# Improbable-AI/walk-these-ways

Hardware: AMD Instinct MI355X
Metric: env-steps/sec (sim+PPO) (higher is better)
Workload: dtype f32

## Files before the change

include/go1ppo.h:

```cpp
#ifndef GO1PPO_H
#define GO1PPO_H
#include <stdint.h>

#ifdef __cplusplus
extern "C" {
#endif

#define GO1PPO_ABI_VERSION 3
#define GO1PPO_MAX_ACTIONS 32

int go1ppo_elu_fwd(void* y, int64_t rows, int cols, int ld, const void* lat, int lat_ld, int npv, const void* wz,
                   int wz_ld, int lat_cols, void* stream);

int go1ppo_elu_bwd(const void* d, int ld_d, const void* h, int ld_h, int64_t rows, int cols, float* bias_grad, void* out,
                   int ld_out, void* stream);

typedef struct {
  const void* mean;
  const void* value;
  const float* std;
  int32_t head_ld, num_actions;
  int64_t rows;
  const int64_t* idx;
  const float* actions;
// ... 3 lines not shown
  const float* advantages;
  const float* returns;
  const float* old_values;
  float clip_param, value_loss_coef, entropy_coef;
  int32_t use_clipped_value_loss;
  void* d_mean;
  void* d_value;
  float* d_std;
  float* d_mean_bias;
  float* d_value_bias;
  float* kl;
  float* value_loss;
  float* surrogate_loss;
} Go1PpoLossArgs;

int go1ppo_loss(const Go1PpoLossArgs* args, void* stream);

int go1ppo_mse(const void* pred, int pred_ld, const float* target, int npv, const int64_t* idx, int64_t rows,
               int64_t num_train, int selective, void* d_pred, float* d_pred_bias, float* train_loss,
               float* test_loss, void* stream);

int go1ppo_wgrad(const void* dz, int ld_dz, const void* h, int ld_h, int64_t rows, int n, int k, float* dW, int ldw,
                 float* bias_grad, void* stream);

#define GO1PPO_TAIL_MAX_LAYERS 4
#define GO1PPO_TAIL_MAX_NETS 3
typedef struct {
  const void* W;
  const void* bias;
  void* out;
  int32_t n_out, k_in, ld_out, elu;
} Go1PpoTailLayer;
typedef struct {
  const void* in;
  int64_t rows;
  int32_t ld_in, num_layers;
  int32_t elu_in, npv;
  const void* latent;
  const void* wz;
  int32_t lat_ld, wz_ld;
  Go1PpoTailLayer layer[GO1PPO_TAIL_MAX_LAYERS];
} Go1PpoTailNet;
typedef struct {
  int32_t num_nets, _pad;
  Go1PpoTailNet net[GO1PPO_TAIL_MAX_NETS];
} Go1PpoTailArgs;
int go1ppo_tail_fwd(const Go1PpoTailArgs* args, void* stream);

typedef struct {
  const void* dz;
  const void* h;
  float* dW;
  float* bias_grad;
  int64_t rows;
  int32_t ld_dz, ld_h, n, k, ldw;
  int32_t chunk_rows, wg_offset;
  int32_t zero_n, zero_k0, zero_k1;
  float* partials;
  int64_t partial_stride;
} Go1PpoWgradProblem;

int go1ppo_wgrad_plan(Go1PpoWgradProblem* host_problems, int count);
int go1ppo_wgrad_batched(const Go1PpoWgradProblem* device_problems, int count, int total_workgroups, void* stream);


int go1ppo_act(const void* mean, const void* value, int head_ld, const float* std, int num_actions, int64_t rows,
               const float* noise, float* actions, float* mu, float* sigma, float* values, float* logp, void* stream);

int go1ppo_store_step(const float* rewards, const uint8_t* dones, const uint8_t* time_outs, const int32_t* env_bins,
                      const float* values, float gamma, int64_t n, float* rewards_out, uint8_t* dones_out,
                      float* env_bins_out, void* stream);

int go1ppo_gae(const float* rewards, const uint8_t* dones, const float* values, const float* last_values, int T, int64_t N,
               float gamma, float lam, float* returns, float* advantages, double* stats, void* stream);

int go1ppo_normalize(float* adv, int64_t n, const double* stats, void* stream);


int go1ppo_ring_snapshot(const float* hist, int64_t ld_hist, int64_t N, int H, int no, void* ring, void* stream);

int go1ppo_ring_step(const float* obs, const float* priv, void* ring_dst, const void* ring_window, int64_t N, int H, int no,
                     int npv, int Kp, void* X, float* obs_store, float* priv_store, void* stream);

int go1ppo_ring_gather(const void* ring, const float* priv_store, const int64_t* idx, int64_t rows, int64_t N, int H, int no,
                       int npv, int Kp, void* X, void* stream);


int go1ppo_opt_partials(void);

int go1ppo_opt_prestep(const float* g, int64_t n, float gscale, float* partial, float* step, float* lr, const float* kl,
                       float kl_scale, float desired_kl, float lr_min, float lr_max, void* stream);

typedef struct {
  int64_t begin, count;
  const void* src;
  int64_t stride;
  int32_t kind, slabs, cols, zero_rows, zero_c0, zero_c1;
} Go1PpoGradPiece;
int go1ppo_grad_reduce(float* g, const Go1PpoGradPiece* device_pieces, int num_pieces, void* stream);
int go1ppo_opt_prestep_pieces(float* g, int64_t n, const Go1PpoGradPiece* device_pieces, int num_pieces, float gscale, float* partial,
                              float* step, float* lr, const float* kl, float kl_scale, float desired_kl, float lr_min, float lr_max,
                              void* stream);

#define GO1PPO_ADAM_MAX_TRANSPOSES 2
typedef struct {
  int32_t num_transposes, _pad;
  struct { int64_t start; int32_t rows, cols; void* dst; } transpose[GO1PPO_ADAM_MAX_TRANSPOSES];
// ... 52 lines not shown
```

walk-these-ways_amd/csrc/go1ppo_gemm.h:

```cpp
#pragma once

#define GEMM_BM 128
#define GEMM_BN 128
#define GEMM_BK 64

typedef __attribute__((address_space(3))) void lds_void_t;
typedef __attribute__((address_space(1))) const void global_cvoid_t;

__device__ __forceinline__ void glds16(const bf16_t* g, bf16_t* lds_wave_base) {
  __builtin_amdgcn_global_load_lds((global_cvoid_t*)g, (lds_void_t*)lds_wave_base, 16, 0, 0);
}

template <int EPI>
__device__ __forceinline__ void gemm_nt_body(const Go1PpoGemmArgs& a, bf16_t (*lds)[2][GEMM_BM * GEMM_BK]) {
  const int lane = threadIdx.x & 63, wave = threadIdx.x >> 6;
  const int nwg = gridDim.x, orig = blockIdx.x;
  const int q = nwg >> 3, r = nwg & 7, xcd = orig & 7;
  const int logical = (xcd < r ? xcd * (q + 1) : r * (q + 1) + (xcd - r) * q) + (orig >> 3);
  const int tiles_n = (a.N + GEMM_BN - 1) / GEMM_BN;
  const int m0 = (logical / tiles_n) * GEMM_BM, n0 = (logical % tiles_n) * GEMM_BN;

  const int srow = lane >> 3;
  const bf16_t* ga[4];
  const bf16_t* gb[4];
// ... 258 lines not shown
}
__device__ __forceinline__ bf16x8_t tn_operand(const TnFrags& f, int i) {
  s16x8_t v = __builtin_shufflevector(f.lo[i], f.hi[i], 0, 1, 2, 3, 4, 5, 6, 7);
  return __builtin_bit_cast(bf16x8_t, v);
}

#define WTN_T 128
#define WTN_STEP 64
#define WTN_BUFS 4
#define WTN_THREADS 512

__device__ __forceinline__ void wgrad_tn_body(const bf16_t* P, int ldp, const bf16_t* Q, int ldq, int64_t m_begin, int steps,
                                              float* C, int ldc, float* bias_row, int N, int K, int n0, int k0,
                                              bf16_t (*lds)[2][WTN_STEP * WTN_T], int zero_n, int zero_k0, int zero_k1, bool slab) {
  const int lane = threadIdx.x & 63, wave = threadIdx.x >> 6;
  const bf16_t* gp[2];
  const bf16_t* gq[2];
  bool vp[2], vq[2];
#pragma unroll
  for (int p = 0; p < 2; p++) {
    const int row = (wave * 2 + p) * 4 + (lane >> 4);
    const int chunk = (lane & 15) ^ (2 * ((row & 3) | (((row >> 3) & 1) << 2)));
    const int cn = n0 + chunk * 8, ck = k0 + chunk * 8;
    vp[p] = cn < N;
    vq[p] = ck < K;
    gp[p] = P + (m_begin + row) * ldp + (vp[p] ? cn : 0);
    gq[p] = Q + (m_begin + row) * ldq + (vq[p] ? ck : 0);
  }
  auto stage_piece = [&](int step, int p, int op) {
    const int buf = step & (WTN_BUFS - 1);
    if (op == 0) { if (vp[p]) glds16(gp[p] + (int64_t)step * WTN_STEP * ldp, &lds[buf][0][(wave * 2 + p) * 4 * WTN_T]); }
    else { if (vq[p]) glds16(gq[p] + (int64_t)step * WTN_STEP * ldq, &lds[buf][1][(wave * 2 + p) * 4 * WTN_T]); }
  };
  auto stage = [&](int step) {
    stage_piece(step, 0, 0); stage_piece(step, 0, 1); stage_piece(step, 1, 0); stage_piece(step, 1, 1);
  };
  const int g = lane >> 4, i16 = lane & 15;
  const int rowoff = (g * 8 + (i16 >> 2)) * 256 + ((i16 & 3) >> 1) * 16 + (i16 & 1) * 8;
  const int swb = 32 * ((i16 >> 2) | ((g & 1) << 2));
  const int wn = wave >> 2, wk = wave & 3;
  int fa[4], fb[2];
#pragma unroll
  for (int f = 0; f < 4; f++) fa[f] = rowoff + (((wn * 64 + f * 16) * 2) ^ swb);
#pragma unroll
  for (int f = 0; f < 2; f++) fb[f] = rowoff + (((wk * 32 + f * 16) * 2) ^ swb);
  f32x4 acc[4][2], bacc[4];
#pragma unroll
  for (int a = 0; a < 4; a++) {
    bacc[a] = f32x4{0.f, 0.f, 0.f, 0.f};
#pragma unroll
    for (int b = 0; b < 2; b++) acc[a][b] = f32x4{0.f, 0.f, 0.f, 0.f};
  }
  const bool do_bias = bias_row && k0 == 0 && wk == 0;
  const s16x8_t ones_bits = {0x3f80, 0x3f80, 0x3f80, 0x3f80, 0x3f80, 0x3f80, 0x3f80, 0x3f80};
  const bf16x8_t ones = __builtin_bit_cast(bf16x8_t, ones_bits);

  const uint32_t lds0 = (uint32_t)(uintptr_t)(lds_void_t*)&lds[0][0][0];
#pragma unroll
  for (int s = 0; s < WTN_BUFS - 1; s++)
    if (s < steps) stage(s);
  for (int s = 0; s < steps; s++) {
    const int younger = steps - 1 - s;
    if (younger >= 2) asm volatile("s_waitcnt vmcnt(8)" ::: "memory");
    else if (younger == 1) asm volatile("s_waitcnt vmcnt(4)" ::: "memory");
    else asm volatile("s_waitcnt vmcnt(0)" ::: "memory");
    __builtin_amdgcn_s_barrier();
    asm volatile("" ::: "memory");
    const bool more = s + WTN_BUFS - 1 < steps;
    const int nxt = s + WTN_BUFS - 1;
    const uint32_t base = lds0 + (uint32_t)(s & (WTN_BUFS - 1)) * (2 * WTN_STEP * WTN_T * 2);
    uint32_t aa[4], ab[2];
#pragma unroll
    for (int f = 0; f < 4; f++) aa[f] = base + fa[f];
#pragma unroll
    for (int f = 0; f < 2; f++) ab[f] = base + WTN_STEP * WTN_T * 2 + fb[f];
    TnFrags f0, f1;
    tn_read<0>(f0, aa, ab);
    tn_read<1>(f1, aa, ab);
    if (more) { stage_piece(nxt, 0, 0); stage_piece(nxt, 0, 1); }
    lds_wait<12>(f0);
#pragma unroll
    for (int a = 0; a < 4; a++) {
#pragma unroll
      for (int b = 0; b < 2; b++)
        acc[a][b] = __builtin_amdgcn_mfma_f32_16x16x32_bf16(tn_operand(f0, a), tn_operand(f0, 4 + b), acc[a][b], 0, 0, 0);
      if (a == 1 && more) stage_piece(nxt, 1, 0);
    }
    if (do_bias) {
#pragma unroll
      for (int a = 0; a < 4; a++) bacc[a] = __builtin_amdgcn_mfma_f32_16x16x32_bf16(tn_operand(f0, a), ones, bacc[a], 0, 0, 0);
    }
    if (more) stage_piece(nxt, 1, 1);
    lds_wait<0>(f1);
#pragma unroll
    for (int a = 0; a < 4; a++)
#pragma unroll
      for (int b = 0; b < 2; b++)
        acc[a][b] = __builtin_amdgcn_mfma_f32_16x16x32_bf16(tn_operand(f1, a), tn_operand(f1, 4 + b), acc[a][b], 0, 0, 0);
    if (do_bias) {
#pragma unroll
      for (int a = 0; a < 4; a++) bacc[a] = __builtin_amdgcn_mfma_f32_16x16x32_bf16(tn_operand(f1, a), ones, bacc[a], 0, 0, 0);
    }
  }
#pragma unroll
  for (int a = 0; a < 4; a++) {
#pragma unroll
    for (int e = 0; e < 4; e++) {
      const int n = n0 + wn * 64 + a * 16 + 4 * g + e;
      if (n >= N) continue;
#pragma unroll
      for (int b = 0; b < 2; b++) {
        const int k = k0 + wk * 32 + b * 16 + i16;
        if (k < K && !(n < zero_n && k >= zero_k0 && k < zero_k1)) {
          if (slab) C[(int64_t)n * ldc + k] = acc[a][b][e];
          else atomicAdd(C + (int64_t)n * ldc + k, acc[a][b][e]);
        }
      }
    }
    if (do_bias && i16 == 0 && n0 + wn * 64 + a * 16 + 4 * g < N) det_put4(bias_row, (wn * 64 + a * 16 + 4 * g) * (int)sizeof(float), bacc[a]);
  }
}

#define WTW_BUF_BYTES (3 * WTN_STEP * WTN_T * 2)
#define WTW_BUFS 3
struct TnFragsW { s16x4_t lo[8], hi[8]; };
template <int KK>
__device__ __forceinline__ void tnw_read(TnFragsW& f, const uint32_t (&aa)[4], const uint32_t (&ab)[4]) {
#pragma unroll
// ... 6 lines not shown
    f.lo[4 + i] = lds_tr<KK * 32 * 256>(ab[i]);
    f.hi[4 + i] = lds_tr<KK * 32 * 256 + 4 * 256>(ab[i]);
  }
}
__device__ __forceinline__ void ldsw_wait_all(TnFragsW& f) {
  asm volatile("s_waitcnt lgkmcnt(0)"
               : "+v"(f.lo[0]), "+v"(f.lo[1]), "+v"(f.lo[2]), "+v"(f.lo[3]), "+v"(f.lo[4]), "+v"(f.lo[5]), "+v"(f.lo[6]), "+v"(f.lo[7]));
  asm volatile("" : "+v"(f.hi[0]), "+v"(f.hi[1]), "+v"(f.hi[2]), "+v"(f.hi[3]), "+v"(f.hi[4]), "+v"(f.hi[5]), "+v"(f.hi[6]), "+v"(f.hi[7]));
}
__device__ __forceinline__ bf16x8_t tnw_operand(const TnFragsW& f, int i) {
  s16x8_t v = __builtin_shufflevector(f.lo[i], f.hi[i], 0, 1, 2, 3, 4, 5, 6, 7);
  return __builtin_bit_cast(bf16x8_t, v);
}

__device__ __forceinline__ void wgrad_tn_body_wide(const bf16_t* P, int ldp, const bf16_t* Q, int ldq, int64_t m_begin, int steps,
                                                   float* C, int ldc, float* bias_row, int N, int K, int n0, int k0, char* lds,
                                                   int zero_n, int zero_k0, int zero_k1, bool slab) {
  const int lane = threadIdx.x & 63, wave = threadIdx.x >> 6;
  const bf16_t* src[6];
  bool ok[6];
  int dst[6];
#pragma unroll
  for (int q = 0; q < 6; q++) {
    const int id = q < 4 ? wave * 4 + q : wave * 2 + (q - 4);
    const int img = q < 4 ? id >> 4 : 2, rb = q < 4 ? id & 15 : id;
    const int row = rb * 4 + (lane >> 4);
    const int chunk = (lane & 15) ^ (2 * ((row & 3) | (((row >> 3) & 1) << 2)));
    const int col = (q < 4 ? n0 + img * 128 : k0) + chunk * 8;
    ok[q] = col < (q < 4 ? N : K);
    src[q] = (q < 4 ? P + (m_begin + row) * ldp : Q + (m_begin + row) * ldq) + (ok[q] ? col : 0);
    dst[q] = img * (WTN_STEP * WTN_T * 2) + rb * 4 * WTN_T * 2;
  }
  auto stage_piece = [&](int step, int buf, int q) {
    if (ok[q]) glds16(src[q] + (int64_t)step * WTN_STEP * (q < 4 ? ldp : ldq), (bf16_t*)(lds + buf * WTW_BUF_BYTES + dst[q]));
  };
  const int g = lane >> 4, i16 = lane & 15;
  const int rowoff = (g * 8 + (i16 >> 2)) * 256 + ((i16 & 3) >> 1) * 16 + (i16 & 1) * 8;
  const int swb = 32 * ((i16 >> 2) | ((g & 1) << 2));
  const int wn = wave >> 1, wk = wave & 1;
  int fa[4], fb[4];
#pragma unroll
  for (int f = 0; f < 4; f++) {
    fa[f] = (wn >> 1) * (WTN_STEP * WTN_T * 2) + rowoff + ((((wn & 1) * 64 + f * 16) * 2) ^ swb);
    fb[f] = 2 * (WTN_STEP * WTN_T * 2) + rowoff + (((wk * 64 + f * 16) * 2) ^ swb);
  }
  f32x4 acc[4][4], bacc[4];
#pragma unroll
  for (int a = 0; a < 4; a++) {
    bacc[a] = f32x4{0.f, 0.f, 0.f, 0.f};
#pragma unroll
    for (int b = 0; b < 4; b++) acc[a][b] = f32x4{0.f, 0.f, 0.f, 0.f};
  }
  const bool do_bias = bias_row && k0 == 0 && wk == 0;
  const s16x8_t ones_bits = {0x3f80, 0x3f80, 0x3f80, 0x3f80, 0x3f80, 0x3f80, 0x3f80, 0x3f80};
  const bf16x8_t ones = __builtin_bit_cast(bf16x8_t, ones_bits);
  const uint32_t lds0 = (uint32_t)(uintptr_t)(lds_void_t*)lds;
#pragma unroll
  for (int s = 0; s < WTW_BUFS - 1; s++)
    if (s < steps) {
#pragma unroll
      for (int q = 0; q < 6; q++) stage_piece(s, s, q);
    }
  int buf = 0;
  for (int s = 0; s < steps; s++) {
    if (s + 1 < steps) asm volatile("s_waitcnt vmcnt(6)" ::: "memory");
    else asm volatile("s_waitcnt vmcnt(0)" ::: "memory");
    __builtin_amdgcn_s_barrier();
    asm volatile("" ::: "memory");
    const bool more = s + WTW_BUFS - 1 < steps;
    const int nxt = s + WTW_BUFS - 1, nbuf = buf == 0 ? WTW_BUFS - 1 : buf - 1;
    const uint32_t base = lds0 + (uint32_t)buf * WTW_BUF_BYTES;
    uint32_t aa[4], ab[4];
#pragma unroll
    for (int f = 0; f < 4; f++) { aa[f] = base + fa[f]; ab[f] = base + fb[f]; }
    TnFragsW f0, f1;
    tnw_read<0>(f0, aa, ab);
    if (more) { stage_piece(nxt, nbuf, 0); stage_piece(nxt, nbuf, 1); stage_piece(nxt, nbuf, 4); }
    ldsw_wait_all(f0);
    tnw_read<1>(f1, aa, ab);
#pragma unroll
    for (int a = 0; a < 4; a++) {
#pragma unroll
      for (int b = 0; b < 4; b++)
        acc[a][b] = __builtin_amdgcn_mfma_f32_16x16x32_bf16(tnw_operand(f0, a), tnw_operand(f0, 4 + b), acc[a][b], 0, 0, 0);
      if (more && a < 3) stage_piece(nxt, nbuf, a == 0 ? 2 : (a == 1 ? 3 : 5));
    }
    if (do_bias) {
#pragma unroll
      for (int a = 0; a < 4; a++) bacc[a] = __builtin_amdgcn_mfma_f32_16x16x32_bf16(tnw_operand(f0, a), ones, bacc[a], 0, 0, 0);
    }
    ldsw_wait_all(f1);
#pragma unroll
    for (int a = 0; a < 4; a++)
#pragma unroll
      for (int b = 0; b < 4; b++)
        acc[a][b] = __builtin_amdgcn_mfma_f32_16x16x32_bf16(tnw_operand(f1, a), tnw_operand(f1, 4 + b), acc[a][b], 0, 0, 0);
    if (do_bias) {
#pragma unroll
      for (int a = 0; a < 4; a++) bacc[a] = __builtin_amdgcn_mfma_f32_16x16x32_bf16(tnw_operand(f1, a), ones, bacc[a], 0, 0, 0);
    }
    buf = buf + 1 == WTW_BUFS ? 0 : buf + 1;
  }
#pragma unroll
  for (int a = 0; a < 4; a++) {
#pragma unroll
    for (int e = 0; e < 4; e++) {
      const int n = n0 + wn * 64 + a * 16 + 4 * g + e;
      if (n >= N) continue;
#pragma unroll
      for (int b = 0; b < 4; b++) {
        const int k = k0 + wk * 64 + b * 16 + i16;
        if (k < K && !(n < zero_n && k >= zero_k0 && k < zero_k1)) {
          if (slab) C[(int64_t)n * ldc + k] = acc[a][b][e];
          else atomicAdd(C + (int64_t)n * ldc + k, acc[a][b][e]);
        }
      }
    }
    if (do_bias && i16 == 0 && n0 + wn * 64 + a * 16 + 4 * g < N) det_put4(bias_row, (wn * 64 + a * 16 + 4 * g) * (int)sizeof(float), bacc[a]);
  }
}
__host__ __device__ __forceinline__ bool wtn_wide(const Go1PpoWgradProblem& P) { return (P.n & 255) == 0 && P.partials != nullptr; }
__host__ __device__ __forceinline__ int wtn_tiles_n(const Go1PpoWgradProblem& P) { return wtn_wide(P) ? P.n >> 8 : (P.n + WTN_T - 1) / WTN_T; }

__device__ __forceinline__ int xcd_remap(int orig, int nwg) {
  const int q = nwg >> 3, r = nwg & 7, xcd = orig & 7;
  return (xcd < r ? xcd * (q + 1) : r * (q + 1) + (xcd - r) * q) + (orig >> 3);
}

__global__ __launch_bounds__(WTN_THREADS, 1) void wgrad_tn_batched_kernel(const Go1PpoWgradProblem* __restrict__ probs, int count) {
  __shared__ __attribute__((aligned(1024))) char lds_raw[WTW_BUFS * WTW_BUF_BYTES];
  static_assert(WTW_BUFS * WTW_BUF_BYTES >= WTN_BUFS * 2 * WTN_STEP * WTN_T * 2, "one LDS block for both tile shapes");
  const int wg = xcd_remap(blockIdx.x, gridDim.x);
  int p = 0;
  while (p + 1 < count && wg >= probs[p + 1].wg_offset) p++;
  const Go1PpoWgradProblem P = probs[p];
  const int local = wg - P.wg_offset;
  const bool wide = wtn_wide(P);
  const int tiles_k = (P.k + WTN_T - 1) / WTN_T, tiles = wtn_tiles_n(P) * tiles_k;
  const int tile = local % tiles, split = local / tiles;
  const int64_t m_begin = (int64_t)split * P.chunk_rows;
  const int64_t m_end = m_begin + P.chunk_rows < P.rows ? m_begin + P.chunk_rows : P.rows;
  const bool slab = P.partials != nullptr;
  float* C = slab ? P.partials + (int64_t)split * P.partial_stride : P.dW;
  const int steps = (int)((m_end - m_begin) / WTN_STEP);
  const int nt = tile / tiles_k, n0 = nt * (wide ? 2 * WTN_T : WTN_T);
  const bool bias = P.bias_grad != nullptr && tile % tiles_k == 0;
  float* bias_slab = det_tn_slab + (int64_t)(p * DET_TN_MAXNT + nt) * DET_TN_MAXS * DET_TN_W;
  float* bias_row = bias ? bias_slab + (int64_t)split * DET_TN_W : nullptr;
  if (wide)
    wgrad_tn_body_wide((const bf16_t*)P.dz, P.ld_dz, (const bf16_t*)P.h, P.ld_h, m_begin, steps, C, P.ldw, bias_row, P.n, P.k,
                       n0, (tile % tiles_k) * WTN_T, lds_raw, P.zero_n, P.zero_k0, P.zero_k1, slab);
  else
    wgrad_tn_body((const bf16_t*)P.dz, P.ld_dz, (const bf16_t*)P.h, P.ld_h, m_begin, steps, C, P.ldw, bias_row, P.n, P.k,
                  n0, (tile % tiles_k) * WTN_T, reinterpret_cast<bf16_t (*)[2][WTN_STEP * WTN_T]>(lds_raw), P.zero_n, P.zero_k0,
                  P.zero_k1, slab);
  if (!bias) return;
  const int splits = (int)((P.rows + P.chunk_rows - 1) / P.chunk_rows);
  if (!det_last(&det_count[DET_TN + p * DET_TN_MAXNT + nt], (unsigned)splits)) return;
  const int width = (wide ? 2 * WTN_T : WTN_T) < P.n - n0 ? (wide ? 2 * WTN_T : WTN_T) : P.n - n0;
  for (int c = threadIdx.x; c < width; c += blockDim.x) {
    float t = 0.f;
#pragma unroll 16
    for (int sp = 0; sp < splits; sp++) t += bias_slab[(int64_t)sp * DET_TN_W + c];
    P.bias_grad[n0 + c] += t;
  }
}

extern "C" int go1ppo_wgrad_tn_plan(Go1PpoWgradProblem* probs, int count) {
  if (!probs || count <= 0) return -1;
  int64_t tile_steps = 0, tiles = 0;
  for (int i = 0; i < count; i++) {
    Go1PpoWgradProblem& P = probs[i];
    if (!P.dz || !P.h || (!P.dW && !P.partials) || (P.partials && P.partial_stride < (int64_t)P.n * P.ldw) || P.rows <= 0 || (P.rows % WTN_STEP) || P.n < 8 || P.k < 8 || (P.n & 7) || (P.k & 7) ||
        (P.ld_dz & 7) || (P.ld_h & 7) || !aligned16(P.dz) || !aligned16(P.h) || P.zero_n < 0 || P.zero_k0 < 0 || P.zero_k1 < P.zero_k0)
      return -1;
    const int64_t t = (int64_t)wtn_tiles_n(P) * ((P.k + WTN_T - 1) / WTN_T);
    tiles += t;
    tile_steps += t * (P.rows / WTN_STEP) * (wtn_wide(P) ? 3 : 2) / 2;
  }
  const int64_t cus = 256;
  int64_t rounds = (tile_steps + cus * 96 - 1) / (cus * 96);
  if (rounds < 1) rounds = 1;
  int64_t chunk_steps = (tile_steps + cus * rounds - 1) / (cus * rounds);
  if (chunk_steps < 4) chunk_steps = 4;
  for (;; chunk_steps++) {
    int total = 0;
    for (int i = 0; i < count; i++) {
      Go1PpoWgradProblem& P = probs[i];
      const int64_t steps = P.rows / WTN_STEP;
      int64_t want = wtn_wide(P) ? chunk_steps * 2 / 3 : chunk_steps;
      if (want < 4) want = 4;
      const int64_t S0 = (steps + want - 1) / want;
      const int64_t cs = (steps + S0 - 1) / S0;
      P.chunk_rows = (int32_t)(cs * WTN_STEP);
      P.wg_offset = total;
      total += (int)((steps + cs - 1) / cs) * wtn_tiles_n(P) * ((P.k + WTN_T - 1) / WTN_T);
    }
    if (total <= cus * rounds || chunk_steps >= 4096) {
      for (int i = 0; i < count; i++) {
        const Go1PpoWgradProblem& P = probs[i];
        if (P.bias_grad && (i >= DET_TN_MAXP || wtn_tiles_n(P) > DET_TN_MAXNT || (P.rows + P.chunk_rows - 1) / P.chunk_rows > DET_TN_MAXS))
          return -2;
      }
      return total;
    }
  }
}

extern "C" int go1ppo_wgrad_tn_batched(const Go1PpoWgradProblem* device_probs, int count, int total_workgroups, void* stream) {
  if (!device_probs || count <= 0 || total_workgroups <= 0) return -1;
  wgrad_tn_batched_kernel<<<dim3((unsigned)total_workgroups), dim3(WTN_THREADS), 0, (hipStream_t)stream>>>(device_probs, count);
  return hipGetLastError() == hipSuccess ? 0 : -9;
}
```

walk-these-ways_amd/go1_gym_learn/ppo_cse/fused.py:

```python
import ctypes
import os

import torch

HEAD = 64
_HERE = os.path.dirname(os.path.abspath(__file__))
_LIB_PATH = os.path.normpath(os.path.join(_HERE, "..", "..", "csrc", "libgo1ppo.so"))
_lib = None


class Go1PpoLibraryMissing(RuntimeError):
    pass


class LossArgs(ctypes.Structure):
    _fields_ = [("mean", ctypes.c_void_p), ("value", ctypes.c_void_p), ("std", ctypes.c_void_p),
                ("head_ld", ctypes.c_int32), ("num_actions", ctypes.c_int32), ("rows", ctypes.c_int64),
                ("idx", ctypes.c_void_p), ("actions", ctypes.c_void_p), ("old_mu", ctypes.c_void_p),
                ("old_sigma", ctypes.c_void_p), ("old_logp", ctypes.c_void_p), ("advantages", ctypes.c_void_p),
                ("returns", ctypes.c_void_p), ("old_values", ctypes.c_void_p),
                ("clip_param", ctypes.c_float), ("value_loss_coef", ctypes.c_float), ("entropy_coef", ctypes.c_float),
                ("use_clipped_value_loss", ctypes.c_int32),
                ("d_mean", ctypes.c_void_p), ("d_value", ctypes.c_void_p), ("d_std", ctypes.c_void_p),
                ("d_mean_bias", ctypes.c_void_p), ("d_value_bias", ctypes.c_void_p), ("kl", ctypes.c_void_p),
                ("value_loss", ctypes.c_void_p), ("surrogate_loss", ctypes.c_void_p)]


class WgradProblem(ctypes.Structure):
    _fields_ = [("dz", ctypes.c_void_p), ("h", ctypes.c_void_p), ("dW", ctypes.c_void_p), ("bias_grad", ctypes.c_void_p),
                ("rows", ctypes.c_int64), ("ld_dz", ctypes.c_int32), ("ld_h", ctypes.c_int32), ("n", ctypes.c_int32),
                ("k", ctypes.c_int32), ("ldw", ctypes.c_int32), ("chunk_rows", ctypes.c_int32), ("wg_offset", ctypes.c_int32),
                ("zero_n", ctypes.c_int32), ("zero_k0", ctypes.c_int32), ("zero_k1", ctypes.c_int32),
                ("partials", ctypes.c_void_p), ("partial_stride", ctypes.c_int64)]


class GradPiece(ctypes.Structure):
    _fields_ = [("begin", ctypes.c_int64), ("count", ctypes.c_int64), ("src", ctypes.c_void_p), ("stride", ctypes.c_int64),
                ("kind", ctypes.c_int32), ("slabs", ctypes.c_int32), ("cols", ctypes.c_int32), ("zero_rows", ctypes.c_int32),
                ("zero_c0", ctypes.c_int32), ("zero_c1", ctypes.c_int32)]


class TailLayer(ctypes.Structure):
    _fields_ = [("W", ctypes.c_void_p), ("bias", ctypes.c_void_p), ("out", ctypes.c_void_p), ("n_out", ctypes.c_int32),
                ("k_in", ctypes.c_int32), ("ld_out", ctypes.c_int32), ("elu", ctypes.c_int32)]


class TailNet(ctypes.Structure):
    _fields_ = [("in_", ctypes.c_void_p), ("rows", ctypes.c_int64), ("ld_in", ctypes.c_int32), ("num_layers", ctypes.c_int32),
                ("elu_in", ctypes.c_int32), ("npv", ctypes.c_int32), ("latent", ctypes.c_void_p), ("wz", ctypes.c_void_p),
                ("lat_ld", ctypes.c_int32), ("wz_ld", ctypes.c_int32),
                ("layer", TailLayer * 4)]


class TailArgs(ctypes.Structure):
    _fields_ = [("num_nets", ctypes.c_int32), ("_pad", ctypes.c_int32), ("net", TailNet * 3)]


class Mlp2Fwd(ctypes.Structure):
    _fields_ = [(n, ctypes.c_void_p) for n in ("x", "W2", "b2", "W3", "b3", "z2", "out")] + [("rows", ctypes.c_int64)] + \
               [(n, ctypes.c_int32) for n in ("ld_x", "ld_z2", "ld_out", "elu_input")]


class Mlp2Bwd(ctypes.Structure):
    _fields_ = [(n, ctypes.c_void_p) for n in ("d_out", "z2", "h", "W2", "W3", "d_z2", "d_x")] + [("rows", ctypes.c_int64)] + \
               [(n, ctypes.c_int32) for n in ("ld_dout", "ld_z2", "ld_h", "ld_dz2", "ld_dx", "_pad")]


MLP2_DIMS = (256, 128, 64)


class GemmArgs(ctypes.Structure):
    _fields_ = [("A", ctypes.c_void_p), ("B", ctypes.c_void_p), ("C", ctypes.c_void_p), ("bias", ctypes.c_void_p),
                ("H", ctypes.c_void_p)] + [(n, ctypes.c_int32) for n in
                                           ("M", "N", "K", "lda", "ldb", "ldc", "ldh", "epilogue", "elu_c0", "elu_c1", "elu_skip_c0", "elu_skip_c1", "bias_bf16", "_pad")]


class _AdamTranspose(ctypes.Structure):
    _fields_ = [("start", ctypes.c_int64), ("rows", ctypes.c_int32), ("cols", ctypes.c_int32), ("dst", ctypes.c_void_p)]


class AdamExtras(ctypes.Structure):
    _fields_ = [("num_transposes", ctypes.c_int32), ("_pad", ctypes.c_int32), ("transpose", _AdamTranspose * 2)]

# ... 117 lines not shown
        assert policy.npv <= HEAD and self.P["Wz"].shape == (self.na, HEAD)
        self._recording, self._batched, self._plans = None, False, {}
        self._grad = grad
        self.defer_grad_sum = False
        self._rec_pieces, self._slab_ws, self._last_pieces = None, {}, {}
        self._wgrad_tn = M % 64 == 0
        self._tails = self._tails_ad = None
        if fused_tails is None:
            fused_tails = M <= int(os.environ.get("GO1_FUSED_TAILS_MAX_ROWS", "2048"))
        self._elu_on_load = not with_grad
        if fused_tails and self._fused_tails_ok():
            nd, na = self.nd, self.na
            eol = self._elu_on_load
            self._tails = (self._tail_args([("adaptation", self.Y1[:, :nd])], with_grad, elu_in=eol),
                           self._tail_args([("actor", self.Y1[:, nd:nd + na]), ("critic", self.Y1[:, nd + na:])], with_grad, elu_in=eol,
                                           latent_for="actor" if eol else None))
            self._tails_ad = self._tail_args([("adaptation", self.Y1d)], with_grad)
        self._mlp2 = (self._tails is None and os.environ.get("GO1_MLP2", "1") == "1" and self.nd == MLP2_DIMS[0] and
                      all(self.depth[n] >= 3 and tuple(self.P[f"{n}.{self.depth[n] - 2}.W"].shape) == (MLP2_DIMS[1], MLP2_DIMS[0])
                          and tuple(self.P[f"{n}.{self.depth[n] - 1}.W"].shape) == (MLP2_DIMS[2], MLP2_DIMS[1]) for n in self.depth)
                      and self.depth["adaptation"] == 3 and self.depth["actor"] == 4 and self.depth["critic"] == 4)
        self._mlp2_cache = {}
        na1, nc1 = int(self.P["actor.1.W"].shape[0]), int(self.P["critic.1.W"].shape[0])
        nt_ok = all(v % 64 == 0 for v in (na1, nc1, self.na, self.n1 - self.nd - self.na)) and \
            all(self.P[k].data_ptr() % 16 == 0 for k in ("actor.1.b", "critic.1.b", "actor.1.W", "critic.1.W"))
        pair_ok = nt_ok and na1 == nc1 and self.na == self.n1 - self.nd - self.na
        self._l1_nt = nt_ok
        self._pair = pair_ok
        self._side = torch.cuda.Stream(device=dev) if two_streams else None
        if with_grad:
            self.X = torch.zeros(M, policy.Kp, **bf)
            self.dH1 = {"adaptation": torch.zeros(M, self.nd, **bf), "actor": torch.zeros(M, self.na, **bf),
                        "critic": torch.zeros(M, self.nc, **bf)}
            self.dY1 = torch.zeros(M, self.n1, **bf)
            self.dZ = {n: {li: torch.zeros_like(z) for li, z in zs.items()} for n, zs in self.Z.items()}
            w1_split = next((b for b in (M // 6144, 4, 2) if b >= 2 and M % b == 0 and (M // b) % 64 == 0), 1)
            self._w1_tmp = torch.zeros(w1_split, self.n1, policy.Kp, **bf)
            self._dgrad_nt = self._mlp2 and nt_ok
            self._WT = {n: torch.zeros(self.P[f"{n}.1.W"].shape[1], self.P[f"{n}.1.W"].shape[0], **bf) for n in ("actor", "critic")} \
                if self._dgrad_nt else None
            self._wt_by_optimizer = False
            self.priv_mask = (self.nd + self.na, policy.K + 1, policy.K + 1 + policy.npv)

    def _elu(self, y, lat=None, lat_cols=0):
        wz = self.P["Wz"] if lat is not None else None
        _chk(self.lib.go1ppo_elu_fwd(y.data_ptr(), y.shape[0], y.shape[1], _ld(y), _ptr(lat), _ld(lat) if lat is not None else 0,
                                     self.pol.npv if lat is not None else 0, _ptr(wz), HEAD, lat_cols, _stream()), "go1ppo_elu_fwd")

    def _elu_bwd(self, d, h, bias_grad, out=None):
        out = d if out is None else out
        _chk(self.lib.go1ppo_elu_bwd(d.data_ptr(), _ld(d), _ptr(h), _ld(h) if h is not None else 0, d.shape[0], d.shape[1],
                                     _ptr(bias_grad), out.data_ptr(), _ld(out), _stream()), "go1ppo_elu_bwd")

    def _wgrad(self, dz, h, gW, gb=None, zero=None):
        n, k = dz.shape[1], h.shape[1]
        assert gW.shape == (n, k) and gW.is_contiguous()
        if self._recording is not None:
            self._recording.append((dz, h, gW, gb, zero))
            return
        if self._batched:
            return
        assert zero is None or zero[0] == 0, "the structural zeros are applied by the batched launch"
        _chk(self.lib.go1ppo_wgrad(dz.data_ptr(), _ld(dz), h.data_ptr(), _ld(h), dz.shape[0], n, k, gW.data_ptr(), k, _ptr(gb),
                                   _stream()), "go1ppo_wgrad")

    def _tail_args(self, nets_and_inputs, keep_intermediates, elu_in=False, latent_for=None):
        a = TailArgs()
        a.num_nets = len(nets_and_inputs)
        for N, (net, h) in zip(a.net, nets_and_inputs):
            d = self.depth[net]
            N.in_, N.rows, N.ld_in, N.num_layers = h.data_ptr(), h.shape[0], _ld(h), d - 1
            N.elu_in = int(bool(elu_in))
            if elu_in and latent_for == net:
                lat, wz = self.Z["adaptation"][self.depth["adaptation"] - 1], self.P["Wz"]
                N.latent, N.wz, N.lat_ld, N.wz_ld, N.npv = lat.data_ptr(), wz.data_ptr(), _ld(lat), HEAD, self.pol.npv
            for li in range(1, d):
                L, W, z = N.layer[li - 1], self.P[f"{net}.{li}.W"], self.Z[net][li]
                last = li == d - 1
                L.W, L.bias = W.data_ptr(), self.P[f"{net}.{li}.b"].data_ptr()
                L.out = z.data_ptr() if (last or keep_intermediates) else None
                L.n_out, L.k_in, L.ld_out, L.elu = W.shape[0], W.shape[1], _ld(z), 0 if last else 1
        return a

    def _fused_tails_ok(self):
        ok = all(self.depth[n] - 1 <= 4 for n in self.depth)
        for n, d in self.depth.items():
            for li in range(1, d):
                r, k = self.P[f"{n}.{li}.W"].shape
                ok = ok and k % 32 == 0 and k <= 512 and r % 16 == 0 and r <= 512
        return ok

    def _tail(self, net, h):
        P, d = self.P, self.depth[net]
        for li in range(1, d):
            z = self.Z[net][li]
            torch.addmm(P[f"{net}.{li}.b"], h, P[f"{net}.{li}.W"].t(), out=z)
            if li < d - 1:
                self._elu(z)
            h = z
        return h

    def forward(self, x):
        nd, na = self.nd, self.na
        if self._mlp2:
            return self._forward_mlp2(x)
        torch.mm(x, self.P["W1"].t(), out=self.Y1)
        if self._tails is not None:
            ta, tac = self._tails
            if not self._elu_on_load:
                self._elu(self.Y1[:, :nd])
            _chk(self.lib.go1ppo_tail_fwd(ctypes.byref(ta), _stream()), "go1ppo_tail_fwd")
# ... 15 lines not shown
        key = ("fwd", key, elu_input)
        if key not in self._mlp2_cache:
            arr = (Mlp2Fwd * len(items))()
            for a, (net, x) in zip(arr, items):
                d = self.depth[net]
                W2, W3, z2, out = self.P[f"{net}.{d - 2}.W"], self.P[f"{net}.{d - 1}.W"], self.Z[net][d - 2], self.Z[net][d - 1]
                a.x, a.W2, a.b2, a.W3, a.b3 = x.data_ptr(), W2.data_ptr(), self.P[f"{net}.{d - 2}.b"].data_ptr(), W3.data_ptr(), self.P[f"{net}.{d - 1}.b"].data_ptr()
                a.z2, a.out, a.rows, a.ld_x, a.ld_z2, a.ld_out, a.elu_input = z2.data_ptr(), out.data_ptr(), x.shape[0], _ld(x), _ld(z2), _ld(out), int(elu_input)
            self._mlp2_cache[key] = (arr, len(items))
        arr, n = self._mlp2_cache[key]
        _chk(self.lib.go1ppo_mlp2_fwd(arr, n, _stream()), "go1ppo_mlp2_fwd")

    def _mlp2_bwd(self, key, items):
        key = ("bwd", key)
        if key not in self._mlp2_cache:
            arr = (Mlp2Bwd * len(items))()
            for a, (net, h, d_x) in zip(arr, items):
                d = self.depth[net]
                d_out, z2, d_z2 = self.dZ[net][d - 1], self.Z[net][d - 2], self.dZ[net][d - 2]
                a.d_out, a.z2, a.h, a.W2, a.W3 = d_out.data_ptr(), z2.data_ptr(), h.data_ptr(), self.P[f"{net}.{d - 2}.W"].data_ptr(), self.P[f"{net}.{d - 1}.W"].data_ptr()
                a.d_z2, a.d_x, a.rows = d_z2.data_ptr(), d_x.data_ptr(), h.shape[0]
                a.ld_dout, a.ld_z2, a.ld_h, a.ld_dz2, a.ld_dx = _ld(d_out), _ld(z2), _ld(h), _ld(d_z2), _ld(d_x)
            self._mlp2_cache[key] = (arr, len(items))
        arr, n = self._mlp2_cache[key]
        _chk(self.lib.go1ppo_mlp2_bwd(arr, n, _stream()), "go1ppo_mlp2_bwd")

    def _forward_mlp2(self, x):
        P, Z, nd, na = self.P, self.Z, self.nd, self.na
        torch.mm(x, P["W1"].t(), out=self.Y1)
        self._mlp2_fwd("adaptation", [("adaptation", self.Y1[:, :nd])])
        latent = Z["adaptation"][2]
        self._elu(self.Y1[:, nd:], latent, na)
        if self._l1_nt and self._pair:
            gemm_nt_pair(self.lib, dict(a=self.Y1[:, nd:nd + na], b=P["actor.1.W"], c=Z["actor"][1], bias=P["actor.1.b"]),
                         dict(a=self.Y1[:, nd + na:], b=P["critic.1.W"], c=Z["critic"][1], bias=P["critic.1.b"]))
        elif self._l1_nt:
            with self._branch():
                gemm_nt(self.lib, self.Y1[:, nd + na:], P["critic.1.W"], Z["critic"][1], P["critic.1.b"])
            gemm_nt(self.lib, self.Y1[:, nd:nd + na], P["actor.1.W"], Z["actor"][1], P["actor.1.b"])
        else:
            with self._branch():
                torch.addmm(P["critic.1.b"], self.Y1[:, nd + na:], P["critic.1.W"].t(), out=Z["critic"][1])
            torch.addmm(P["actor.1.b"], self.Y1[:, nd:nd + na], P["actor.1.W"].t(), out=Z["actor"][1])
        self._join()
        self._mlp2_fwd("ac", [("actor", Z["actor"][1]), ("critic", Z["critic"][1])])
        return Z["actor"][3], Z["critic"][3], latent

    def _backward_mlp2(self, x):
        nd, na = self.nd, self.na
        P, G, Z, dZ, Y1, dY1, dH1 = self.P, self.G, self.Z, self.dZ, self.Y1, self.dY1, self.dH1
        cols = {"adaptation": slice(0, nd), "actor": slice(nd, nd + na), "critic": slice(nd + na, self.n1)}
        self._mlp2_bwd("ac", [("actor", Z["actor"][1], dZ["actor"][1]), ("critic", Z["critic"][1], dZ["critic"][1])])
        for net in ("actor", "critic"):
            self._wgrad(dZ[net][3], Z[net][2], G[f"{net}.3.W"], None)
            self._wgrad(dZ[net][2], Z[net][1], G[f"{net}.2.W"], G[f"{net}.2.b"])
            self._wgrad(dZ[net][1], Y1[:, cols[net]], G[f"{net}.1.W"], G[f"{net}.1.b"])
        if self._dgrad_nt and self._pair and self._wt_by_optimizer:
            gemm_nt_pair(self.lib, dict(a=dZ["actor"][1], b=self._WT["actor"], c=dY1[:, cols["actor"]], elu_bwd_of=Y1[:, cols["actor"]]),
                         dict(a=dZ["critic"][1], b=self._WT["critic"], c=dY1[:, cols["critic"]], elu_bwd_of=Y1[:, cols["critic"]]))
        elif self._dgrad_nt:
            with self._branch():
                if not self._wt_by_optimizer:
                    self._WT["critic"].copy_(P["critic.1.W"].t())
                gemm_nt(self.lib, dZ["critic"][1], self._WT["critic"], dY1[:, cols["critic"]], elu_bwd_of=Y1[:, cols["critic"]])
            if not self._wt_by_optimizer:
                self._WT["actor"].copy_(P["actor.1.W"].t())
            gemm_nt(self.lib, dZ["actor"][1], self._WT["actor"], dY1[:, cols["actor"]], elu_bwd_of=Y1[:, cols["actor"]])
        else:
            with self._branch():
                torch.mm(dZ["critic"][1], P["critic.1.W"], out=dH1["critic"])
                self._elu_bwd(dH1["critic"], Y1[:, cols["critic"]], None, out=dY1[:, cols["critic"]])
            torch.mm(dZ["actor"][1], P["actor.1.W"], out=dH1["actor"])
            self._elu_bwd(dH1["actor"], Y1[:, cols["actor"]], None, out=dY1[:, cols["actor"]])
        latent, dlat = Z["adaptation"][2], dZ["adaptation"][2]
        dA1 = dY1[:, cols["actor"]]
        self._wgrad(dA1, latent, G["Wz"])
        torch.mm(dA1, P["Wz"], out=dlat)
        self._mlp2_bwd("adaptation", [("adaptation", Y1[:, :nd], dY1[:, :nd])])
        self._wgrad(dlat, Z["adaptation"][1], G["adaptation.2.W"], G["adaptation.2.b"])
        self._wgrad(dZ["adaptation"][1], Y1[:, :nd], G["adaptation.1.W"], G["adaptation.1.b"])
        self._join()
        self._big_wgrad(dY1, x, G["W1"], self._w1_tmp)

    def _forward_adaptation_mlp2(self, x):
        torch.mm(x, self.P["W1"][:self.nd].t(), out=self.Y1d)
        self._mlp2_fwd("adaptation_only", [("adaptation", self.Y1d)])
        return self.Z["adaptation"][2]

    def _backward_adaptation_mlp2(self, x):
        nd, d, G, Z, dZ = self.nd, self.dH1["adaptation"], self.G, self.Z, self.dZ
        self._mlp2_bwd("adaptation_only", [("adaptation", self.Y1d, d)])
        self._wgrad(dZ["adaptation"][2], Z["adaptation"][1], G["adaptation.2.W"], None)
        self._wgrad(dZ["adaptation"][1], self.Y1d, G["adaptation.1.W"], G["adaptation.1.b"])
        self._big_wgrad(d, x, G["W1"][:nd], self._w1_tmp[:, :nd], own_kernel=self._wgrad_tn)

    def adam_transposes(self):
        if not getattr(self, "_dgrad_nt", False):
            return []
        out = []
        for n in ("actor", "critic"):
            i = self.pol.index[f"{n}.1.W"]
            rows, cols = self.pol.blocks[i][1]
            out.append((self.pol.offsets[i], rows, cols, self._WT[n]))
        return out

    def refresh_transposes(self):
        if getattr(self, "_dgrad_nt", False):
            for n in ("actor", "critic"):
                self._WT[n].copy_(self.P[f"{n}.1.W"].t())

    def _branch(self):
        if self._side is None:
            import contextlib
            return contextlib.nullcontext()
        self._side.wait_stream(torch.cuda.current_stream())
        self._forked = True
        return torch.cuda.stream(self._side)

    def _join(self):
        if self._side is not None and getattr(self, "_forked", False):
            torch.cuda.current_stream().wait_stream(self._side)
            self._forked = False

    def forward_adaptation(self, x):
        if self._mlp2:
            return self._forward_adaptation_mlp2(x)
        torch.mm(x, self.P["W1"][:self.nd].t(), out=self.Y1d)
        self._elu(self.Y1d)
        if self._tails_ad is not None:
            _chk(self.lib.go1ppo_tail_fwd(ctypes.byref(self._tails_ad), _stream()), "go1ppo_tail_fwd")
            return self.Z["adaptation"][self.depth["adaptation"] - 1]
        return self._tail("adaptation", self.Y1d)

    def _tail_bwd(self, net, h0, dh0, head_bias_done=True):
        P, G, d = self.P, self.G, self.depth[net]
        for li in range(d - 1, 0, -1):
            dz = self.dZ[net][li]
            h_in = self.Z[net][li - 1] if li > 1 else h0
            gb = None if (li == d - 1 and head_bias_done) else G[f"{net}.{li}.b"]
            self._wgrad(dz, h_in, G[f"{net}.{li}.W"], gb)
            out = self.dZ[net][li - 1] if li > 1 else dh0
            torch.mm(dz, P[f"{net}.{li}.W"], out=out)
            if li > 1:
                self._elu_bwd(out, h_in, None)

    def _big_wgrad(self, dY, x, gW, tmp, own_kernel=False):
        zr, zc0, zc1 = self.priv_mask
        zr = min(zr, gW.shape[0])
        if own_kernel:
            self._wgrad(dY, x, gW, zero=(zr, zc0, zc1))
            return
        b = tmp.shape[0]
        if b == 1 or not tmp.is_contiguous():
            torch.mm(dY.t(), x, out=tmp[0])
            part, count, stride = tmp[0], 1, gW.numel()
        else:
            torch.bmm(dY.view(b, dY.shape[0] // b, dY.shape[1]).transpose(1, 2), x.view(b, x.shape[0] // b, x.shape[1]), out=tmp)
            part, count, stride = tmp, b, tmp.stride(0)
        assert gW.is_contiguous() and part.stride(-1) == 1 and part.stride(-2) == gW.shape[1]
        if self._rec_pieces is not None:
            self._rec_pieces.append(dict(begin=self._grad_offset(gW), count=gW.numel(), src=part, stride=stride, kind=2, slabs=count,
                                         cols=gW.shape[1], zero=(zr, zc0, zc1)))

    def _grad_offset(self, view):
        off = (view.data_ptr() - self._grad.data_ptr()) // 4
        assert view.dtype == torch.float32 and view.is_contiguous() and 0 <= off and off + view.numel() <= self._grad.numel()
        return int(off)

    def last_pieces(self, kind):
        return self._last_pieces.get(kind)

    def _run_planned(self, key, fn):
        if key not in self._plans:
            self._recording, self._rec_pieces = [], []
            fn()
            rec, self._recording = self._recording, None
            pieces, self._rec_pieces = self._rec_pieces, None
            tab = (WgradProblem * len(rec))()
            for P, (dz, h, gW, gb, zero) in zip(tab, rec):
                P.dz, P.h, P.dW, P.bias_grad = dz.data_ptr(), h.data_ptr(), gW.data_ptr(), _ptr(gb)
                if zero is not None:
                    P.zero_n, P.zero_k0, P.zero_k1 = zero
                P.rows, P.ld_dz, P.ld_h, P.n, P.k, P.ldw = dz.shape[0], _ld(dz), _ld(h), dz.shape[1], h.shape[1], gW.shape[1]
            tn = self._wgrad_tn and all(P.rows % 64 == 0 and P.n % 8 == 0 and P.k % 8 == 0 for P in tab)
            plan = self.lib.go1ppo_wgrad_tn_plan if tn else self.lib.go1ppo_wgrad_plan
            if tn:
                for P, (dz, h, gW, gb, zero) in zip(tab, rec):
                    P.partials, P.partial_stride = 16, gW.numel()
            total = plan(tab, len(rec))
            if total <= 0:
                raise RuntimeError(f"go1ppo_wgrad_plan failed with code {total}")
            if tn:
                for j, (P, (dz, h, gW, gb, zero)) in enumerate(zip(tab, rec)):
                    S = -(-P.rows // P.chunk_rows)
                    ws = self._slab_ws.get((key[0], j))
                    if ws is None or tuple(ws.shape) != (S, gW.numel()):
                        ws = self._slab_ws[(key[0], j)] = torch.zeros(S, gW.numel(), device=gW.device, dtype=torch.float32)
                    P.partials, P.partial_stride = ws.data_ptr(), gW.numel()
                    pieces.append(dict(begin=self._grad_offset(gW), count=gW.numel(), src=ws, stride=gW.numel(), kind=1, slabs=S, cols=gW.shape[1],
                                       zero=(0, 0, 0)))
                if plan(tab, len(rec)) != total:
                    raise RuntimeError("go1ppo_wgrad_tn_plan: the plan changed with the slab buffers attached")
            dev = torch.frombuffer(bytearray(bytes(tab)), dtype=torch.uint8).to(self.Y1.device)
            ptab = None
            if pieces:
                pieces.sort(key=lambda q: q["begin"])
                arr = (GradPiece * len(pieces))()
                end = 0
                for A, q in zip(arr, pieces):
                    assert q["begin"] >= end and q["begin"] % 8 == 0 and q["count"] % 8 == 0 and q["stride"] % 8 == 0, "slab pieces: ascending, disjoint, multiples of 8"
                    end = q["begin"] + q["count"]
                    A.begin, A.count, A.src, A.stride, A.kind, A.slabs, A.cols = q["begin"], q["count"], q["src"].data_ptr(), q["stride"], q["kind"], q["slabs"], q["cols"]
                    A.zero_rows, A.zero_c0, A.zero_c1 = q["zero"]
                ptab = (torch.frombuffer(bytearray(bytes(arr)), dtype=torch.uint8).to(self.Y1.device), len(pieces), [q["src"] for q in pieces])
            self._plans[key] = (dev, len(rec), total, rec, tn, ptab)
        else:
            self._batched = True
            try:
                fn()
            finally:
                self._batched = False
        dev, count, total, _, tn, ptab = self._plans[key]
        launch = self.lib.go1ppo_wgrad_tn_batched if tn else self.lib.go1ppo_wgrad_batched
        _chk(launch(dev.data_ptr(), count, total, _stream()), "go1ppo_wgrad_batched")
        self._last_pieces[key[0]] = None
        if ptab is None:
            return
        if self.defer_grad_sum:
            self._last_pieces[key[0]] = ptab[:2]
        else:
            _chk(self.lib.go1ppo_grad_reduce(self._grad.data_ptr(), ptab[0].data_ptr(), ptab[1], _stream()), "go1ppo_grad_reduce")

    def backward(self, x):
        self._run_planned(("ppo", x.data_ptr()), lambda: (self._backward_mlp2 if self._mlp2 else self._backward)(x))

# ... 167 lines not shown
```

Measured before the change: 5.161 million.

## Skip padded rows/cols in batched TN weight-gradient tiles and rebalance split planning

Adds n_use/k_use fields so weight-gradient problems whose outputs are padded (actor/critic last layer, Wz, adaptation.2) only compute the live region. Waves whose tile falls entirely in padding skip the MFMA work and only keep staging loads. The planner now balances row splits by tile column cost, not tile count. The risk: narrowing rows to int32 changes the ABI, and padded gradient entries are left uncomputed and must already be zero or unused.

```diff
diff --git a/include/go1ppo.h b/include/go1ppo.h
--- a/include/go1ppo.h
+++ b/include/go1ppo.h
@@ -79,7 +79,8 @@
   const void* h;
   float* dW;
   float* bias_grad;
-  int64_t rows;
+  int32_t rows;
+  int16_t n_use, k_use;
   int32_t ld_dz, ld_h, n, k, ldw;
   int32_t chunk_rows, wg_offset;
   int32_t zero_n, zero_k0, zero_k1;
diff --git a/walk-these-ways_amd/csrc/go1ppo_gemm.h b/walk-these-ways_amd/csrc/go1ppo_gemm.h
--- a/walk-these-ways_amd/csrc/go1ppo_gemm.h
+++ b/walk-these-ways_amd/csrc/go1ppo_gemm.h
@@ -334,6 +334,7 @@
     for (int b = 0; b < 2; b++) acc[a][b] = f32x4{0.f, 0.f, 0.f, 0.f};
   }
   const bool do_bias = bias_row && k0 == 0 && wk == 0;
+  const bool live = n0 + wn * 64 < N && k0 + wk * 32 < K;
   const s16x8_t ones_bits = {0x3f80, 0x3f80, 0x3f80, 0x3f80, 0x3f80, 0x3f80, 0x3f80, 0x3f80};
   const bf16x8_t ones = __builtin_bit_cast(bf16x8_t, ones_bits);
 
@@ -356,6 +357,10 @@
     for (int f = 0; f < 4; f++) aa[f] = base + fa[f];
 #pragma unroll
     for (int f = 0; f < 2; f++) ab[f] = base + WTN_STEP * WTN_T * 2 + fb[f];
+    if (!live) {
+      if (more) stage(nxt);
+      continue;
+    }
     TnFrags f0, f1;
     tn_read<0>(f0, aa, ab);
     tn_read<1>(f1, aa, ab);
@@ -468,6 +473,7 @@
     for (int b = 0; b < 4; b++) acc[a][b] = f32x4{0.f, 0.f, 0.f, 0.f};
   }
   const bool do_bias = bias_row && k0 == 0 && wk == 0;
+  const bool live = n0 + wn * 64 < N && k0 + wk * 64 < K;
   const s16x8_t ones_bits = {0x3f80, 0x3f80, 0x3f80, 0x3f80, 0x3f80, 0x3f80, 0x3f80, 0x3f80};
   const bf16x8_t ones = __builtin_bit_cast(bf16x8_t, ones_bits);
   const uint32_t lds0 = (uint32_t)(uintptr_t)(lds_void_t*)lds;
@@ -489,6 +495,14 @@
     uint32_t aa[4], ab[4];
 #pragma unroll
     for (int f = 0; f < 4; f++) { aa[f] = base + fa[f]; ab[f] = base + fb[f]; }
+    if (!live) {
+      if (more) {
+#pragma unroll
+        for (int q = 0; q < 6; q++) stage_piece(nxt, nbuf, q);
+      }
+      buf = buf + 1 == WTW_BUFS ? 0 : buf + 1;
+      continue;
+    }
     TnFragsW f0, f1;
     tnw_read<0>(f0, aa, ab);
     if (more) { stage_piece(nxt, nbuf, 0); stage_piece(nxt, nbuf, 1); stage_piece(nxt, nbuf, 4); }
@@ -535,8 +549,15 @@
     if (do_bias && i16 == 0 && n0 + wn * 64 + a * 16 + 4 * g < N) det_put4(bias_row, (wn * 64 + a * 16 + 4 * g) * (int)sizeof(float), bacc[a]);
   }
 }
-__host__ __device__ __forceinline__ bool wtn_wide(const Go1PpoWgradProblem& P) { return (P.n & 255) == 0 && P.partials != nullptr; }
-__host__ __device__ __forceinline__ int wtn_tiles_n(const Go1PpoWgradProblem& P) { return wtn_wide(P) ? P.n >> 8 : (P.n + WTN_T - 1) / WTN_T; }
+__host__ __device__ __forceinline__ int wtn_n(const Go1PpoWgradProblem& P) { return P.n_use > 0 && P.n_use < P.n ? (P.n_use + 7) & ~7 : P.n; }
+__host__ __device__ __forceinline__ int wtn_k(const Go1PpoWgradProblem& P) { return P.k_use > 0 && P.k_use < P.k ? (P.k_use + 7) & ~7 : P.k; }
+__host__ __device__ __forceinline__ bool wtn_wide(const Go1PpoWgradProblem& P) { return (wtn_n(P) & 255) == 0 && P.partials != nullptr; }
+__host__ __device__ __forceinline__ int wtn_tiles_n(const Go1PpoWgradProblem& P) { return wtn_wide(P) ? wtn_n(P) >> 8 : (wtn_n(P) + WTN_T - 1) / WTN_T; }
+__host__ __device__ __forceinline__ int wtn_tiles_k(const Go1PpoWgradProblem& P) { return (wtn_k(P) + WTN_T - 1) / WTN_T; }
+__host__ __device__ __forceinline__ int wtn_tile_cols(const Go1PpoWgradProblem& P) {
+  const int tn = wtn_wide(P) ? 2 * WTN_T : WTN_T, n = wtn_n(P), k = wtn_k(P);
+  return (n < tn ? n : tn) + (k < WTN_T ? k : WTN_T);
+}
 
 __device__ __forceinline__ int xcd_remap(int orig, int nwg) {
   const int q = nwg >> 3, r = nwg & 7, xcd = orig & 7;
@@ -552,7 +573,8 @@
   const Go1PpoWgradProblem P = probs[p];
   const int local = wg - P.wg_offset;
   const bool wide = wtn_wide(P);
-  const int tiles_k = (P.k + WTN_T - 1) / WTN_T, tiles = wtn_tiles_n(P) * tiles_k;
+  const int N = wtn_n(P), K = wtn_k(P);
+  const int tiles_k = wtn_tiles_k(P), tiles = wtn_tiles_n(P) * tiles_k;
   const int tile = local % tiles, split = local / tiles;
   const int64_t m_begin = (int64_t)split * P.chunk_rows;
   const int64_t m_end = m_begin + P.chunk_rows < P.rows ? m_begin + P.chunk_rows : P.rows;
@@ -564,16 +586,16 @@
   float* bias_slab = det_tn_slab + (int64_t)(p * DET_TN_MAXNT + nt) * DET_TN_MAXS * DET_TN_W;
   float* bias_row = bias ? bias_slab + (int64_t)split * DET_TN_W : nullptr;
   if (wide)
-    wgrad_tn_body_wide((const bf16_t*)P.dz, P.ld_dz, (const bf16_t*)P.h, P.ld_h, m_begin, steps, C, P.ldw, bias_row, P.n, P.k,
+    wgrad_tn_body_wide((const bf16_t*)P.dz, P.ld_dz, (const bf16_t*)P.h, P.ld_h, m_begin, steps, C, P.ldw, bias_row, N, K,
                        n0, (tile % tiles_k) * WTN_T, lds_raw, P.zero_n, P.zero_k0, P.zero_k1, slab);
   else
-    wgrad_tn_body((const bf16_t*)P.dz, P.ld_dz, (const bf16_t*)P.h, P.ld_h, m_begin, steps, C, P.ldw, bias_row, P.n, P.k,
+    wgrad_tn_body((const bf16_t*)P.dz, P.ld_dz, (const bf16_t*)P.h, P.ld_h, m_begin, steps, C, P.ldw, bias_row, N, K,
                   n0, (tile % tiles_k) * WTN_T, reinterpret_cast<bf16_t (*)[2][WTN_STEP * WTN_T]>(lds_raw), P.zero_n, P.zero_k0,
                   P.zero_k1, slab);
   if (!bias) return;
-  const int splits = (int)((P.rows + P.chunk_rows - 1) / P.chunk_rows);
+  const int splits = (int)(((int64_t)P.rows + P.chunk_rows - 1) / P.chunk_rows);
   if (!det_last(&det_count[DET_TN + p * DET_TN_MAXNT + nt], (unsigned)splits)) return;
-  const int width = (wide ? 2 * WTN_T : WTN_T) < P.n - n0 ? (wide ? 2 * WTN_T : WTN_T) : P.n - n0;
+  const int width = (wide ? 2 * WTN_T : WTN_T) < N - n0 ? (wide ? 2 * WTN_T : WTN_T) : N - n0;
   for (int c = threadIdx.x; c < width; c += blockDim.x) {
     float t = 0.f;
 #pragma unroll 16
@@ -584,33 +606,32 @@
 
 extern "C" int go1ppo_wgrad_tn_plan(Go1PpoWgradProblem* probs, int count) {
   if (!probs || count <= 0) return -1;
-  int64_t tile_steps = 0, tiles = 0;
+  int64_t tile_cols = 0;
   for (int i = 0; i < count; i++) {
     Go1PpoWgradProblem& P = probs[i];
     if (!P.dz || !P.h || (!P.dW && !P.partials) || (P.partials && P.partial_stride < (int64_t)P.n * P.ldw) || P.rows <= 0 || (P.rows % WTN_STEP) || P.n < 8 || P.k < 8 || (P.n & 7) || (P.k & 7) ||
-        (P.ld_dz & 7) || (P.ld_h & 7) || !aligned16(P.dz) || !aligned16(P.h) || P.zero_n < 0 || P.zero_k0 < 0 || P.zero_k1 < P.zero_k0)
+        (P.ld_dz & 7) || (P.ld_h & 7) || !aligned16(P.dz) || !aligned16(P.h) || P.zero_n < 0 || P.zero_k0 < 0 || P.zero_k1 < P.zero_k0 ||
+        P.n_use < 0 || P.n_use > P.n || P.k_use < 0 || P.k_use > P.k)
       return -1;
-    const int64_t t = (int64_t)wtn_tiles_n(P) * ((P.k + WTN_T - 1) / WTN_T);
-    tiles += t;
-    tile_steps += t * (P.rows / WTN_STEP) * (wtn_wide(P) ? 3 : 2) / 2;
-  }
-  const int64_t cus = 256;
-  int64_t rounds = (tile_steps + cus * 96 - 1) / (cus * 96);
+    tile_cols += ((int64_t)wtn_tiles_k(P) * wtn_n(P) + (int64_t)wtn_tiles_n(P) * wtn_k(P)) * (P.rows / WTN_STEP);
+  }
+  const int64_t cus = 256, unit = 2 * WTN_T;
+  int64_t rounds = (tile_cols + cus * 96 * unit - 1) / (cus * 96 * unit);
   if (rounds < 1) rounds = 1;
-  int64_t chunk_steps = (tile_steps + cus * rounds - 1) / (cus * rounds);
+  int64_t chunk_steps = (tile_cols + cus * rounds * unit - 1) / (cus * rounds * unit);
   if (chunk_steps < 4) chunk_steps = 4;
   for (;; chunk_steps++) {
     int total = 0;
     for (int i = 0; i < count; i++) {
       Go1PpoWgradProblem& P = probs[i];
       const int64_t steps = P.rows / WTN_STEP;
-      int64_t want = wtn_wide(P) ? chunk_steps * 2 / 3 : chunk_steps;
+      int64_t want = chunk_steps * unit / wtn_tile_cols(P);
       if (want < 4) want = 4;
       const int64_t S0 = (steps + want - 1) / want;
       const int64_t cs = (steps + S0 - 1) / S0;
       P.chunk_rows = (int32_t)(cs * WTN_STEP);
       P.wg_offset = total;
-      total += (int)((steps + cs - 1) / cs) * wtn_tiles_n(P) * ((P.k + WTN_T - 1) / WTN_T);
+      total += (int)((steps + cs - 1) / cs) * wtn_tiles_n(P) * wtn_tiles_k(P);
     }
     if (total <= cus * rounds || chunk_steps >= 4096) {
       for (int i = 0; i < count; i++) {
diff --git a/walk-these-ways_amd/go1_gym_learn/ppo_cse/fused.py b/walk-these-ways_amd/go1_gym_learn/ppo_cse/fused.py
--- a/walk-these-ways_amd/go1_gym_learn/ppo_cse/fused.py
+++ b/walk-these-ways_amd/go1_gym_learn/ppo_cse/fused.py
@@ -28,7 +28,7 @@
 
 class WgradProblem(ctypes.Structure):
     _fields_ = [("dz", ctypes.c_void_p), ("h", ctypes.c_void_p), ("dW", ctypes.c_void_p), ("bias_grad", ctypes.c_void_p),
-                ("rows", ctypes.c_int64), ("ld_dz", ctypes.c_int32), ("ld_h", ctypes.c_int32), ("n", ctypes.c_int32),
+                ("rows", ctypes.c_int32), ("n_use", ctypes.c_int16), ("k_use", ctypes.c_int16), ("ld_dz", ctypes.c_int32), ("ld_h", ctypes.c_int32), ("n", ctypes.c_int32),
                 ("k", ctypes.c_int32), ("ldw", ctypes.c_int32), ("chunk_rows", ctypes.c_int32), ("wg_offset", ctypes.c_int32),
                 ("zero_n", ctypes.c_int32), ("zero_k0", ctypes.c_int32), ("zero_k1", ctypes.c_int32),
                 ("partials", ctypes.c_void_p), ("partial_stride", ctypes.c_int64)]
@@ -252,11 +252,12 @@
         _chk(self.lib.go1ppo_elu_bwd(d.data_ptr(), _ld(d), _ptr(h), _ld(h) if h is not None else 0, d.shape[0], d.shape[1],
                                      _ptr(bias_grad), out.data_ptr(), _ld(out), _stream()), "go1ppo_elu_bwd")
 
-    def _wgrad(self, dz, h, gW, gb=None, zero=None):
+    def _wgrad(self, dz, h, gW, gb=None, zero=None, use=None):
         n, k = dz.shape[1], h.shape[1]
         assert gW.shape == (n, k) and gW.is_contiguous()
         if self._recording is not None:
             self._recording.append((dz, h, gW, gb, zero))
+            self._recording_use.append(use)
             return
         if self._batched:
             return
@@ -378,7 +379,7 @@
         cols = {"adaptation": slice(0, nd), "actor": slice(nd, nd + na), "critic": slice(nd + na, self.n1)}
         self._mlp2_bwd("ac", [("actor", Z["actor"][1], dZ["actor"][1]), ("critic", Z["critic"][1], dZ["critic"][1])])
         for net in ("actor", "critic"):
-            self._wgrad(dZ[net][3], Z[net][2], G[f"{net}.3.W"], None)
+            self._wgrad(dZ[net][3], Z[net][2], G[f"{net}.3.W"], None, use=(self.pol.out_dims[net], 0))
             self._wgrad(dZ[net][2], Z[net][1], G[f"{net}.2.W"], G[f"{net}.2.b"])
             self._wgrad(dZ[net][1], Y1[:, cols[net]], G[f"{net}.1.W"], G[f"{net}.1.b"])
         if self._dgrad_nt and self._pair and self._wt_by_optimizer:
@@ -400,10 +401,10 @@
             self._elu_bwd(dH1["actor"], Y1[:, cols["actor"]], None, out=dY1[:, cols["actor"]])
         latent, dlat = Z["adaptation"][2], dZ["adaptation"][2]
         dA1 = dY1[:, cols["actor"]]
-        self._wgrad(dA1, latent, G["Wz"])
+        self._wgrad(dA1, latent, G["Wz"], use=(0, self.pol.npv))
         torch.mm(dA1, P["Wz"], out=dlat)
         self._mlp2_bwd("adaptation", [("adaptation", Y1[:, :nd], dY1[:, :nd])])
-        self._wgrad(dlat, Z["adaptation"][1], G["adaptation.2.W"], G["adaptation.2.b"])
+        self._wgrad(dlat, Z["adaptation"][1], G["adaptation.2.W"], G["adaptation.2.b"], use=(self.pol.npv, 0))
         self._wgrad(dZ["adaptation"][1], Y1[:, :nd], G["adaptation.1.W"], G["adaptation.1.b"])
         self._join()
         self._big_wgrad(dY1, x, G["W1"], self._w1_tmp)
@@ -416,7 +417,7 @@
     def _backward_adaptation_mlp2(self, x):
         nd, d, G, Z, dZ = self.nd, self.dH1["adaptation"], self.G, self.Z, self.dZ
         self._mlp2_bwd("adaptation_only", [("adaptation", self.Y1d, d)])
-        self._wgrad(dZ["adaptation"][2], Z["adaptation"][1], G["adaptation.2.W"], None)
+        self._wgrad(dZ["adaptation"][2], Z["adaptation"][1], G["adaptation.2.W"], None, use=(self.pol.npv, 0))
         self._wgrad(dZ["adaptation"][1], self.Y1d, G["adaptation.1.W"], G["adaptation.1.b"])
         self._big_wgrad(d, x, G["W1"][:nd], self._w1_tmp[:, :nd], own_kernel=self._wgrad_tn)
 
@@ -498,15 +499,17 @@
 
     def _run_planned(self, key, fn):
         if key not in self._plans:
-            self._recording, self._rec_pieces = [], []
+            self._recording, self._recording_use, self._rec_pieces = [], [], []
             fn()
-            rec, self._recording = self._recording, None
+            rec, uses, self._recording, self._recording_use = self._recording, self._recording_use, None, None
             pieces, self._rec_pieces = self._rec_pieces, None
             tab = (WgradProblem * len(rec))()
-            for P, (dz, h, gW, gb, zero) in zip(tab, rec):
+            for P, (dz, h, gW, gb, zero), use in zip(tab, rec, uses):
                 P.dz, P.h, P.dW, P.bias_grad = dz.data_ptr(), h.data_ptr(), gW.data_ptr(), _ptr(gb)
                 if zero is not None:
                     P.zero_n, P.zero_k0, P.zero_k1 = zero
+                if use is not None:
+                    P.n_use, P.k_use = use
                 P.rows, P.ld_dz, P.ld_h, P.n, P.k, P.ldw = dz.shape[0], _ld(dz), _ld(h), dz.shape[1], h.shape[1], gW.shape[1]
             tn = self._wgrad_tn and all(P.rows % 64 == 0 and P.n % 8 == 0 and P.k % 8 == 0 for P in tab)
             plan = self.lib.go1ppo_wgrad_tn_plan if tn else self.lib.go1ppo_wgrad_plan
```

Measured after the change: 5.083 million, median of 2. 1.5% lower.
